# ZhangYY12345/aswStereoMatch

Measured on AMD Instinct MI355X. Metric: disparity Mpix/s, 1920x1080 D=128 classic bilateral ASW (computeAdaptiveWeight), higher is better.
Workload: dtype f64; 1 GPU; 1920x1080 D=128 win=15 bilateral, 8 frames/GPU/step resident in HBM, cost volume kept; candidates=129, parallelism=frames sharded, no collective, ranks=1, backend=none

## Files before the change

### aswstereomatch_amd/csrc/k_bilateral_xq.hip

```cpp
#include <stdlib.h>

#include <algorithm>
#include <cmath>

#include "asw_device.h"
#include "asw_internal.h"

namespace {

constexpr int HH = 7;
constexpr int KS = 2 * HH + 1;
constexpr int PXW = 64;
constexpr int LWC = PXW + 2 * HH;
constexpr int NSTEP = KS + 3;
constexpr int RING = 5;
constexpr int URI = 3;
constexpr int CROW = 6;
static_assert(KS % URI == 0 && CROW % URI == 0, "whole bodies");
constexpr int NCELLCOL = NSTEP + 3;
constexpr int LW8 = 80;
constexpr int LWP = 80;

template <int NW>
struct XqCfg {
    static constexpr int NWAVE = NW;
    static constexpr int NTHR = 64 * NW;
    static constexpr int NJ = 4 * NW;
    static constexpr int NPOS = PXW + 4 * NJ;
    static constexpr int RWC = NPOS + 2 * HH;
    static constexpr int NFIN = 4 * NJ;
    static constexpr int RW8 = (RWC + 3) / 4 * 4;
    static constexpr int NROWS = (KS + NW - 1) / NW;
    static constexpr int RWP = (RWC + 3) / 4 * 4;
    static constexpr int LROW = RING * PXW + LWP;
    static constexpr int RROW = 2 * NPOS + RWP;
    static constexpr int LGRAY = RING * PXW;
    static constexpr int RGRAY = 2 * NPOS;
    static constexpr int OFF_LB = 0;
    static constexpr int OFF_RB = OFF_LB + KS * LROW * 4;
    static constexpr int OFF_L8 = OFF_RB + KS * RROW * 4;
    static constexpr int OFF_R8 = OFF_L8 + KS * LW8;
    static constexpr int OFF_CELL = OFF_R8 + KS * RW8;
    static constexpr int OFF_E64 = 0;
    static constexpr int OFF_PART = (NFIN + 1) * PXW * 8;
    static constexpr int LDS_TOTAL = std::max((OFF_CELL + NCELLCOL * KS * 2 + 15) / 16 * 16, OFF_PART + NW * PXW * 12);
    static_assert(LDS_TOTAL <= (NW == 8 ? 80 : 53) * 1024, "two (NW = 8) / three (NW = 4) workgroups per CU");
    static_assert(OFF_RB % 16 == 0 && (LROW * 4) % 16 == 0 && (RROW * 4) % 16 == 0 && (NPOS * 4) % 16 == 0 && (LGRAY * 4) % 16 == 0, "b128 alignment");
    static_assert(NPOS % 64 == 0, "positions are staged in whole wavefront passes");
};
#define XQ_CONSTS(NW)                                                                                                           \
    typedef XqCfg<NW> Cfg;                                                                                                       \
    constexpr int NWAVE = Cfg::NWAVE, NTHR = Cfg::NTHR, NJ = Cfg::NJ, NPOS = Cfg::NPOS, RWC = Cfg::RWC, NFIN = Cfg::NFIN, RW8 = Cfg::RW8,      \
                  NROWS = Cfg::NROWS, LROW = Cfg::LROW, RROW = Cfg::RROW, LGRAY = Cfg::LGRAY, RGRAY = Cfg::RGRAY,               \
                  OFF_LB = Cfg::OFF_LB, OFF_RB = Cfg::OFF_RB, OFF_L8 = Cfg::OFF_L8, OFF_R8 = Cfg::OFF_R8, OFF_CELL = Cfg::OFF_CELL,  \
                  LDS_TOTAL = Cfg::LDS_TOTAL, OFF_E64 = Cfg::OFF_E64, OFF_PART = Cfg::OFF_PART;                                  \
    (void)NWAVE; (void)NTHR; (void)NJ; (void)NPOS; (void)RWC; (void)NFIN; (void)RW8; (void)NROWS; (void)LROW; (void)RROW; (void)LGRAY;  \
    (void)RGRAY; (void)OFF_LB; (void)OFF_RB; (void)OFF_L8; (void)OFF_R8; (void)OFF_CELL; (void)LDS_TOTAL; (void)OFF_E64; (void)OFF_PART;

struct XqParams {
    int H, W, minD;
    int tile0;
};

__device__ __forceinline__ double cost_sample(uint32_t gl, uint32_t gr, uint32_t hi0)
{
    const uint32_t c = __builtin_amdgcn_sad_u16(gl, gr, 0u);
    return __builtin_bit_cast(double, (uint64_t)c | ((uint64_t)hi0 << 32));
}

template <int NW>
__device__ __forceinline__ void cell_at(const unsigned char* smem, int idx, int& dxw, int& dyw, int& cls256)
{
    XQ_CONSTS(NW)
    const uint32_t u = reinterpret_cast<const uint16_t*>(smem + OFF_CELL)[idx];
    dxw = (int)(u & 15u) - 8;
    dyw = (int)((u >> 4) & 15u) - 8;
    cls256 = (int)(u >> 8) << 8;
}

template <int NW> struct Staged { float v[XqCfg<NW>::NROWS][1 + XqCfg<NW>::NPOS / 64]; };

template <int NW>
__device__ __forceinline__ void stage_issue(int Kn, const float* __restrict__ lut, const unsigned char* smem, int wave, int lane,
                                            uint32_t ppack, Staged<NW>& st)
{
    XQ_CONSTS(NW)
    const uint8_t* sL8 = smem + OFF_L8;
    const uint8_t* sR8 = smem + OFF_R8;
#pragma unroll
    for (int rr = 0; rr < NROWS; rr++) {
        const int ky = wave + NWAVE * rr;
        if (ky >= KS) break;
        int dxw, dyw, cls;
        if (Kn < KS) {
            cell_at<NW>(smem, (Kn + 3) * KS + ky, dxw, dyw, cls);
            const int nb = sL8[(HH + dyw) * LW8 + (lane + HH + dxw)];
            st.v[rr][0] = lut_at(lut, __builtin_amdgcn_sad_u16(nb, sL8[HH * LW8 + lane + HH], cls));
        }
#pragma unroll
        for (int r3 = 0; r3 < NPOS / 64; r3++) {
            const int b = lane & 3;
            cell_at<NW>(smem, (Kn - b + 3) * KS + ky, dxw, dyw, cls);
            const int pc = (int)((ppack >> (8 * r3)) & 255u) + HH;
            const int ctr = sR8[HH * RW8 + pc];
            const int nb = sR8[(HH + dyw) * RW8 + pc + dxw];
            st.v[rr][1 + r3] = lut_at(lut, __builtin_amdgcn_sad_u16(nb, ctr, cls));
        }
    }
}

template <int NW>
__device__ __forceinline__ void stage_commit(int Kn, unsigned char* smem, int wave, int lane, const Staged<NW>& st)
{
    XQ_CONSTS(NW)
    float* sWL = reinterpret_cast<float*>(smem + OFF_LB) + (Kn % RING) * PXW;
    float* sWR = reinterpret_cast<float*>(smem + OFF_RB) + (Kn & 1) * NPOS;
#pragma unroll
    for (int rr = 0; rr < NROWS; rr++) {
        const int ky = wave + NWAVE * rr;
        if (ky >= KS) break;
        if (Kn < KS) sWL[ky * LROW + lane] = st.v[rr][0];
#pragma unroll
        for (int r3 = 0; r3 < NPOS / 64; r3++) sWR[ky * RROW + lane + 64 * r3] = st.v[rr][1 + r3];
    }
}

template <int NW>
__device__ __forceinline__ void stage_weights(int Kn, const float* __restrict__ lut, unsigned char* smem, int wave, int lane,
                                              uint32_t ppack)
{
    Staged<NW> st;
    stage_issue<NW>(Kn, lut, smem, wave, lane, ppack, st);
    stage_commit<NW>(Kn, smem, wave, lane, st);
}

__device__ __forceinline__ int fresh_lane()
{
    int l;
    asm volatile("v_mbcnt_lo_u32_b32 %0, -1, 0\n\tv_mbcnt_hi_u32_b32 %0, -1, %0" : "=&v"(l));
    return l;
}
template <int NPOS>
__device__ __forceinline__ uint32_t pack_positions(int lane, int pclamp_lo, int pclamp_hi)
{
    uint32_t ppack = 0;
#pragma unroll
    for (int r3 = 0; r3 < NPOS / 64; r3++) ppack |= (uint32_t)min(max(lane + 64 * r3, pclamp_lo), pclamp_hi) << (8 * r3);
    asm volatile("" : "+v"(ppack));
    return ppack;
}
template <int NW> constexpr int UWAVE = NW - 1;
template <bool ON> struct USums {};
template <> struct USums<true> { double num = 0.0, den = 0.0; };

template <int NW, int K, bool EDGE, bool WRAPW, bool COMMIT, bool RIGHT, bool LASTW, bool FRESH>
__device__ __forceinline__ void run_step(unsigned char* smem, int g, int qrel, int qrel2, int xabs, int dbase, int dbase2,
                                         int W, int x0, int posmin, double (&num)[4][4], double (&den)[4][4], USums<LASTW>& us,
                                         int wave, int lane, const Staged<NW>& st)
{
    static_assert(!LASTW || (!EDGE && !WRAPW), "the last-candidate units live in a plain wavefront of an interior tile");
    XQ_CONSTS(NW)
    constexpr int BLO = K > KS - 1 ? K - (KS - 1) : 0;
    constexpr int BHI = K < 3 ? K : 3;
    constexpr int DLO = 0 - BHI, DHI = 3 - BLO;
    const uint32_t* sLd = reinterpret_cast<const uint32_t*>(smem + OFF_LB) + LGRAY;
    const uint32_t* sRd = reinterpret_cast<const uint32_t*>(smem + OFF_RB) + RGRAY;

    int iL[7], iR[7];
    if constexpr (EDGE) {
#pragma unroll
        for (int dl = DLO; dl <= DHI; dl++) {
            const int lc = min(max(xabs + dl + K - HH, 0), W - 1);
            const int rc = RIGHT ? lc + ((dl > 0 ? dbase2 : dbase) - dl) : lc - ((dl < 0 ? dbase2 : dbase) + dl);
            iL[dl + 3] = min(max(lc - (x0 - HH), 0), LWC - 1);
            iR[dl + 3] = min(max(rc - (posmin - HH), 0), RWC - 1);
        }
    }
    typedef __attribute__((address_space(3))) const unsigned char lds_u8;
    lds_u8* bL = (lds_u8*)smem + OFF_LB + 16 * g;
    lds_u8* bR = (lds_u8*)smem + OFF_RB + 4 * qrel;
    lds_u8* bR2 = (lds_u8*)smem + OFF_RB + 4 * qrel2;
    lds_u8* uL = nullptr; lds_u8* uW = nullptr; lds_u8* uG = nullptr;
    if constexpr (FRESH) {
        static_assert(!EDGE, "interior tiles");
        const int l2 = fresh_lane();
        g = (l2 & 7) | ((l2 >> 2) & 8);
        const int jl = 4 * wave + ((l2 >> 3) & 3);
        qrel = RIGHT ? 4 * g + 4 * jl : 4 * g + 4 * (NJ - jl);
        qrel2 = jl == 0 ? (RIGHT ? 4 * g + 4 * NJ : 4 * g) : qrel;
        bL = (lds_u8*)smem + OFF_LB + 16 * g;
        bR = (lds_u8*)smem + OFF_RB + 4 * qrel;
        bR2 = (lds_u8*)smem + OFF_RB + 4 * qrel2;
    }
    if constexpr (LASTW) {
        static_assert(FRESH, "g is this step's own");
        const int a = (fresh_lane() >> 3) & 3;
        const int slot = a == 0 ? (K + RING) % RING : a == 1 ? (K - 1 + RING) % RING : a == 2 ? (K - 2 + RING) % RING : (K - 3 + RING) % RING;
        uL = (lds_u8*)smem + OFF_LB + 16 * g + 4 * a + 4 * PXW * slot;
        uW = (lds_u8*)smem + OFF_RB + 16 * g + (RIGHT ? 16 * NJ : 0) + 4 * a + 4 * (K & 1) * NPOS;
        uG = (lds_u8*)smem + OFF_RB + 16 * g + (RIGHT ? 16 * NJ : 0);
        asm("" : "+v"(uL), "+v"(uW), "+v"(uG));
    }
    uint32_t hi0[7];
#pragma unroll
    for (int i = 0; i < 7; i++) asm volatile("v_mov_b32 %0, 0" : "=v"(hi0[i]));
    constexpr int UR = EDGE ? 1 : URI;
    auto rows = [&](int ky0, int nbody) {
#pragma unroll 1
        for (int it = 0; it < nbody; it++) {
#pragma unroll
            for (int u = 0; u < UR; u++) {
                lds_u8* rL = bL + u * 4 * LROW;
                lds_u8* rR = bR + u * 4 * RROW;
                lds_u8* rR2 = bR2 + u * 4 * RROW;
                double c[7];
                uint32_t glU = 0;
                (void)glU;
                if constexpr (!EDGE) {
                    const uint32_t gr = *(const __attribute__((address_space(3))) uint32_t*)(rR + 4 * (RGRAY + K));
                    uint32_t gr2 = gr;
                    if constexpr (WRAPW && (RIGHT ? DHI > 0 : DLO < 0)) gr2 = *(const __attribute__((address_space(3))) uint32_t*)(rR2 + 4 * (RGRAY + K));
                    constexpr int E0 = (K + DLO) & ~3, NQ = (K + DHI - E0 + 4) / 4;
                    static_assert(E0 >= 0 && E0 + 4 * NQ + 4 * 15 <= LWP, "the quads stay inside a tile row");
                    typedef uint32_t u32x4 __attribute__((ext_vector_type(4)));
                    const __attribute__((address_space(3))) u32x4* pl4 = (const __attribute__((address_space(3))) u32x4*)(rL + 4 * (LGRAY + E0));
                    uint32_t glv[4 * NQ];
#pragma unroll
                    for (int i = 0; i < NQ; i++) {
                        u32x4 t = pl4[i];
                        asm("" : "+v"(t));
                        glv[4 * i] = t.x; glv[4 * i + 1] = t.y; glv[4 * i + 2] = t.z; glv[4 * i + 3] = t.w;
                    }
#pragma unroll
                    for (int dl = DLO; dl <= DHI; dl++) c[dl + 3] = cost_sample(glv[K + dl - E0], (RIGHT ? dl > 0 : dl < 0) ? gr2 : gr, hi0[dl + 3]);
                    static_assert(DLO <= 0 && DHI >= 0, "diagonal 0 is in use in every step");
                    glU = glv[K - E0];
                } else {
                    const int ky = ky0 + it * UR + u;
#pragma unroll
                    for (int dl = DLO; dl <= DHI; dl++) c[dl + 3] = cost_sample(sLd[ky * LROW + iL[dl + 3]], sRd[ky * RROW + iR[dl + 3]], hi0[dl + 3]);
                }
                typedef float f32x4 __attribute__((ext_vector_type(4)));
                typedef __attribute__((address_space(3))) const f32x4 lds_f32x4;
                const f32x4 wr4 = *(lds_f32x4*)(rR + 4 * (K & 1) * NPOS);
                typedef float f32x2 __attribute__((ext_vector_type(2)));
                f32x2 wrp[2] = {{wr4.x, wr4.y}, {wr4.z, wr4.w}};
                asm("" : "+v"(wrp[1]));
                f32x2 wr2p[2] = {wrp[0], wrp[1]};
                if constexpr ((WRAPW || EDGE) && (RIGHT ? BLO <= 2 : BHI >= 1)) {
                    const f32x4 w2 = *(lds_f32x4*)(rR2 + 4 * (K & 1) * NPOS);
                    wr2p[0] = f32x2{w2.x, w2.y};
                    wr2p[1] = f32x2{w2.z, w2.w};
                    asm("" : "+v"(wr2p[1]));
                }
#pragma unroll
                for (int b = BLO; b <= BHI; b++) {
                    const f32x4 wl4 = *(lds_f32x4*)(rL + 4 * ((K - b) % RING) * PXW);
                    float ab[4];
#pragma unroll
                    for (int a = 0; a < 4; a += 2) {
                        const f32x2 wl2 = {wl4[a], wl4[a + 1]};
                        const bool w0 = RIGHT ? b < a : a < b, w1 = RIGHT ? b < a + 1 : a + 1 < b;
                        const f32x2 s0 = (w0 ? wr2p : wrp)[b >> 1], s1 = (w1 ? wr2p : wrp)[b >> 1];
                        f32x2 wrb;
                        if (w0 == w1) wrb = (b & 1) ? __builtin_shufflevector(s0, s0, 1, 1) : __builtin_shufflevector(s0, s0, 0, 0);
                        else wrb = f32x2{s0[b & 1], s1[b & 1]};
                        const f32x2 pr = wl2 * wrb;
                        ab[a] = pr.x; ab[a + 1] = pr.y;
                    }
#pragma unroll
                    for (int a = 0; a < 4; a++) {
                        const double abd = (double)ab[a];
                        num[a][b] = __builtin_fma(abd, c[a - b + 3], num[a][b]);
                        den[a][b] = den[a][b] + abd;
                    }
                }
                if constexpr (LASTW) {
                    constexpr int E0 = (K + DLO) & ~3;
                    (void)E0;
                    typedef __attribute__((address_space(3))) const uint32_t lds_u32;
                    typedef __attribute__((address_space(3))) const float lds_f32;
                    const float wlU = *(lds_f32*)(uL + u * 4 * LROW);
                    const float wrU = *(lds_f32*)(uW + u * 4 * RROW);
                    const uint32_t grU = *(lds_u32*)(uG + u * 4 * RROW + 4 * (RGRAY + K));
                    const double abU = (double)(wlU * wrU);
                    us.num = __builtin_fma(abU, cost_sample(glU, grU, hi0[3]), us.num);
                    us.den = us.den + abU;
                    asm volatile("" :: "v"(us.num), "v"(us.den));
                }
#pragma unroll
                for (int b = BLO; b <= BHI; b++)
                    asm volatile("" :: "v"(num[0][b]), "v"(num[1][b]), "v"(num[2][b]), "v"(num[3][b]),
                                       "v"(den[0][b]), "v"(den[1][b]), "v"(den[2][b]), "v"(den[3][b]) : "memory");
                __builtin_amdgcn_sched_barrier(0);
            }
            bL += UR * 4 * LROW;
            bR += UR * 4 * RROW;
            asm("" : "+v"(bL), "+v"(bR));
            if constexpr (WRAPW || EDGE) {
                bR2 += UR * 4 * RROW;
                asm("" : "+v"(bR2));
            }
            if constexpr (LASTW) {
                uL += UR * 4 * LROW;
                uW += UR * 4 * RROW;
                uG += UR * 4 * RROW;
                asm("" : "+v"(uL), "+v"(uW), "+v"(uG));
            }
        }
    };
    if constexpr (COMMIT) {
        rows(0, CROW / UR);
        stage_commit<NW>(K + 1, smem, wave, FRESH ? fresh_lane() : lane, st);
        rows(CROW, (KS - CROW) / UR);
    } else {
        rows(0, KS / UR);
    }
}

template <int NW, bool EDGE, bool WRAPW, int ABL, bool RIGHT, bool LASTW = false, bool FRESH = false>
__device__ __forceinline__ void run_all_steps(unsigned char* smem, const float* __restrict__ lut, int wave, int lane,
                                              uint32_t ppack, int g, int qrel, int qrel2, int xabs, int dbase, int dbase2,
                                              int W, int x0, int posmin, double (&num)[4][4], double (&den)[4][4], USums<LASTW>& us, int pclamp_lo = 0,
                                              int pclamp_hi = 0)
{
    Staged<NW> st;
#define ASW_XQ_STEP(KK)                                                                                        \
    if (!(ABL & 1) && (KK) + 1 < NSTEP) {                                                                        \
        if constexpr (FRESH) { lane = fresh_lane(); ppack = pack_positions<XqCfg<NW>::NPOS>(lane, pclamp_lo, pclamp_hi); }  \
        if constexpr (EDGE) stage_weights<NW>((KK) + 1, lut, smem, wave, lane, ppack);   \
        else stage_issue<NW>((KK) + 1, lut, smem, wave, lane, ppack, st);                      \
    }                                                                                                           \
    run_step<NW, (KK), EDGE, WRAPW, (!EDGE && !(ABL & 1) && (KK) + 1 < NSTEP), RIGHT, LASTW, FRESH>(smem, g, qrel, qrel2, xabs, dbase, dbase2, W, x0, \
                                                                           posmin, num, den, us, wave, lane, st); \
    if (!(ABL & 2) || (KK) == NSTEP - 1) __syncthreads();
    ASW_XQ_STEP(0) ASW_XQ_STEP(1) ASW_XQ_STEP(2) ASW_XQ_STEP(3) ASW_XQ_STEP(4) ASW_XQ_STEP(5)
    ASW_XQ_STEP(6) ASW_XQ_STEP(7) ASW_XQ_STEP(8) ASW_XQ_STEP(9) ASW_XQ_STEP(10) ASW_XQ_STEP(11)
    ASW_XQ_STEP(12) ASW_XQ_STEP(13) ASW_XQ_STEP(14) ASW_XQ_STEP(15) ASW_XQ_STEP(16) ASW_XQ_STEP(17)
#undef ASW_XQ_STEP
}

template <int NW, bool EDGE, int ABL, bool RIGHT, bool LASTC = false>
__global__ __launch_bounds__(64 * NW) __attribute__((amdgpu_waves_per_eu(NW == 8 ? 4 : 3, NW == 8 ? 4 : 3))) void k_asw_bilateral_xq(
    XqParams p, const uint8_t* __restrict__ gL, const uint8_t* __restrict__ gR, const int4* __restrict__ cells,
    const float* __restrict__ lut, float* __restrict__ vol, double* __restrict__ bestE, float* __restrict__ bestD,
    float* __restrict__ disp)
{
    XQ_CONSTS(NW)
    static_assert(!(EDGE && LASTC), "the border tiles cannot host the last-candidate units");
    __shared__ __align__(16) unsigned char smem[LDS_TOTAL];
    const int tid = threadIdx.x, lane = tid & 63, wave = __builtin_amdgcn_readfirstlane(tid >> 6);
    const int H = p.H, W = p.W;
    const int x0 = (p.tile0 + blockIdx.x) * PXW, y = blockIdx.y;
    const int posmin = RIGHT ? x0 + p.minD : x0 - p.minD - 4 * NJ;

    {
        uint8_t* sL8 = smem + OFF_L8;
        uint8_t* sR8 = smem + OFF_R8;
        uint32_t* sLd = reinterpret_cast<uint32_t*>(smem + OFF_LB) + Cfg::LGRAY;
        uint32_t* sRd = reinterpret_cast<uint32_t*>(smem + OFF_RB) + Cfg::RGRAY;
        for (int i = tid; i < KS * LWC; i += NTHR) {
            const int r = i / LWC, c = i - r * LWC;
            const int yy = min(max(y - HH + r, 0), H - 1), xx = min(max(x0 - HH + c, 0), W - 1);
            const int v = gL[(size_t)yy * W + xx];
            sL8[r * LW8 + c] = (uint8_t)v;
            sLd[r * Cfg::LROW + c] = (uint32_t)v;
        }
        for (int i = tid; i < KS * RWC; i += NTHR) {
            const int r = i / RWC, c = i - r * RWC;
            const int yy = min(max(y - HH + r, 0), H - 1), xx = min(max(posmin - HH + c, 0), W - 1);
            const int v = gR[(size_t)yy * W + xx];
            sR8[r * RW8 + c] = (uint8_t)v;
            sRd[r * Cfg::RROW + c] = (uint32_t)v;
        }
        if constexpr (LASTC) {
            float* sWL = reinterpret_cast<float*>(smem + OFF_LB);
            for (int i = tid; i < KS * 3 * PXW; i += NTHR) {
                const int r = i / (3 * PXW), c = i - r * (3 * PXW);
                sWL[r * Cfg::LROW + 2 * PXW + c] = 0.0f;
            }
        }
        uint16_t* sCell = reinterpret_cast<uint16_t*>(smem + OFF_CELL);
        for (int i = tid; i < NCELLCOL * KS; i += NTHR) {
            const int4 ci = cells[i];
            sCell[i] = (uint16_t)((uint32_t)(ci.x + 8) | ((uint32_t)(ci.y + 8) << 4) | ((uint32_t)(ci.z >> 8) << 8));
        }
    }
    __syncthreads();

    const int g = (lane & 7) | ((lane >> 2) & 8);
    const int jl = 4 * wave + ((lane >> 3) & 3);
    const int qrel = RIGHT ? 4 * g + 4 * jl : 4 * g + 4 * (NJ - jl);
    const int qrel2 = jl == 0 ? (RIGHT ? 4 * g + 4 * NJ : 4 * g) : qrel;
    const int xabs = x0 + 4 * g;
    const int dbase = p.minD + 4 * jl;
    const int dbase2 = jl == 0 ? p.minD + 4 * NJ : dbase;
    const int pclamp_lo = min(max(0 - posmin, 0), NPOS - 1), pclamp_hi = min(max(W - 1 - posmin, 0), NPOS - 1);
    static_assert(NPOS <= 256, "a clamped position fits a byte");
    const uint32_t ppack = pack_positions<NPOS>(lane, pclamp_lo, pclamp_hi);

    double num[4][4], den[4][4];
#pragma unroll
    for (int a = 0; a < 4; a++)
#pragma unroll
        for (int b = 0; b < 4; b++) { num[a][b] = 0.0; den[a][b] = 0.0; }

    USums<LASTC> us;
    USums<false> none;
    stage_weights<NW>(0, lut, smem, wave, lane, ppack);
    __syncthreads();
    if (EDGE || wave == 0)
        run_all_steps<NW, EDGE, true, ABL, RIGHT, false, LASTC>(smem, lut, wave, lane, ppack, g, qrel, qrel2, xabs, dbase, dbase2, W,
                                                                 x0, posmin, num, den, none, pclamp_lo, pclamp_hi);
    else if (LASTC && wave == UWAVE<NW>)
        run_all_steps<NW, EDGE, false, ABL, RIGHT, LASTC, LASTC>(smem, lut, UWAVE<NW>, lane, ppack, g, qrel, qrel2, xabs, dbase, dbase2, W,
                                                                  x0, posmin, num, den, us, pclamp_lo, pclamp_hi);
    else
        run_all_steps<NW, EDGE, false, ABL, RIGHT, false, LASTC>(smem, lut, wave, lane, ppack, g, qrel, qrel2, xabs, dbase, dbase2, W,
                                                                  x0, posmin, num, den, none, pclamp_lo, pclamp_hi);

    int le = lane;
    asm volatile("" : "+v"(le));
    const int ge = (le & 7) | ((le >> 2) & 8), jle = 4 * wave + ((le >> 3) & 3);
    const int cb = 4 * jle, cb2 = jle == 0 ? 4 * NJ : cb;
    double* sE = reinterpret_cast<double*>(smem + OFF_E64);
#pragma unroll
    for (int a = 0; a < 4; a++)
#pragma unroll
        for (int b = 0; b < 4; b++) {
            const int c = RIGHT ? (b < a ? cb2 : cb) + b - a : (a < b ? cb2 : cb) + a - b;
            sE[c * PXW + 4 * ge + a] = __builtin_ldexp(num[a][b], 954) / __builtin_ldexp(den[a][b], -120);
        }
    if constexpr (LASTC)
        if (wave == UWAVE<NW>) sE[NFIN * PXW + 4 * ge + ((le >> 3) & 3)] = __builtin_ldexp(us.num, 954) / __builtin_ldexp(us.den, -120);
    __syncthreads();
    const int px = lane, part = wave;
    const int x = x0 + px;
    double be = 1.7976931348623157e308;
    float bd = 0.0f;
    if (x < W) {
        for (int c = 16 * part; c < 16 * part + 16; c++) {
            const double E = sE[c * PXW + px];
            if (vol) vol[((size_t)c * H + y) * W + x] = (float)E;
            if (E < be) { be = E; bd = (float)(p.minD + c); }
        }
    }
    double* sPE = reinterpret_cast<double*>(smem + OFF_PART);
    float* sPD = reinterpret_cast<float*>(smem + OFF_PART + NWAVE * PXW * 8);
    sPE[part * PXW + px] = be;
    sPD[part * PXW + px] = bd;
    __syncthreads();
    if (wave == 0 && x < W) {
        double e = 1.7976931348623157e308;
        float d = 0.0f;
#pragma unroll
        for (int q = 0; q < NWAVE; q++) {
            const double eq = sPE[q * PXW + px];
            if (eq < e) { e = eq; d = sPD[q * PXW + px]; }
        }
        if constexpr (LASTC) {
            const double eq = sE[NFIN * PXW + px];
            if (vol) vol[((size_t)NFIN * H + y) * W + x] = (float)eq;
            if (eq < e) { e = eq; d = (float)(p.minD + NFIN); }
        }
        if (LASTC || disp) {
            disp[(size_t)y * W + x] = d;
        } else {
            bestE[(size_t)y * W + x] = e;
            bestD[(size_t)y * W + x] = d;
        }
    }
}

}

int bilateral_xq_candidates(int nwave) { return 16 * nwave; }

bool bilateral_xq_lut_ok(const float* lut, size_t n)
{
    double mn = 0, mx = 0;
    for (size_t i = 0; i < n; i++) {
        const double v = lut[i];
        if (!(v >= 0)) return false;
        if (v > 0 && (mn == 0 || v < mn)) mn = v;
        if (v > mx) mx = v;
    }
    return mn * mn >= std::ldexp(1.0, -68) && mx * mx < std::ldexp(1.0, 128 - 2 * XQ_LUT_SCALE_LOG2 - 1);
}

namespace {
template <int NW>
int launch_xq_t(hipStream_t s, hipStream_t s_border, const uint8_t* gL, const uint8_t* gR, int H, int W, int minD, const int4* cells,
                const float* lut, float* vol, double* bestE, float* bestD, float* disp, bool right, bool last)
{
    const int ntiles = (W + PXW - 1) / PXW;
    const dim3 blk(64 * NW);
    if (right) {
        if ((ntiles - 1) * PXW + minD > W - 1) return ASW_ERR_BAD_ARGUMENT;
        XqParams pe{H, W, minD, 0};
        hipLaunchKernelGGL((k_asw_bilateral_xq<NW, true, 0, true>), dim3(1, H), blk, 0, s_border, pe, gL, gR, cells, lut, vol,
                           bestE, bestD, last ? nullptr : disp);
        if (ntiles > 1) {
            XqParams pi{H, W, minD, 1};
            if (last)
                hipLaunchKernelGGL((k_asw_bilateral_xq<NW, false, 0, true, true>), dim3(ntiles - 1, H), blk, 0, s, pi, gL, gR, cells,
                                   lut, vol, bestE, bestD, disp);
            else
                hipLaunchKernelGGL((k_asw_bilateral_xq<NW, false, 0, true>), dim3(ntiles - 1, H), blk, 0, s, pi, gL, gR, cells, lut,
                                   vol, bestE, bestD, disp);
        }
        ASW_HIP_TRY(hipGetLastError());
        return ASW_OK;
    }
    const int n_int = W >= PXW + HH ? std::min(ntiles, (W - PXW - HH) / PXW + 1) : 0;
#ifdef ASW_XQ_ABLATION
    int abl = 0;
    if (const char* e = getenv("ASW_XQ_ABLATE")) abl = atoi(e) & 3;
    auto ki = abl == 0 ? k_asw_bilateral_xq<NW, false, 0, false> : abl == 1 ? k_asw_bilateral_xq<NW, false, 1, false>
            : abl == 2 ? k_asw_bilateral_xq<NW, false, 2, false> : k_asw_bilateral_xq<NW, false, 3, false>;
#else
    auto ki = k_asw_bilateral_xq<NW, false, 0, false>;
#endif
    auto ke = k_asw_bilateral_xq<NW, true, 0, false>;
    if (n_int > 0) {
        XqParams p{H, W, minD, 0};
        if (last)
            hipLaunchKernelGGL((k_asw_bilateral_xq<NW, false, 0, false, true>), dim3(n_int, H), blk, 0, s, p, gL, gR, cells, lut, vol,
                               bestE, bestD, disp);
        else
            hipLaunchKernelGGL(ki, dim3(n_int, H), blk, 0, s, p, gL, gR, cells, lut, vol, bestE, bestD, disp);
    }
    if (ntiles > n_int) {
        XqParams p{H, W, minD, n_int};
        hipLaunchKernelGGL(ke, dim3(ntiles - n_int, H), blk, 0, s_border, p, gL, gR, cells, lut, vol, bestE, bestD,
                           last ? nullptr : disp);
    }
    ASW_HIP_TRY(hipGetLastError());
    return ASW_OK;
}
}

int launch_bilateral_xq(hipStream_t s, hipStream_t s_border, int nwave, const uint8_t* gL, const uint8_t* gR, int H, int W, int minD,
                        const int4* cells, const float* lut, float* vol, double* bestE, float* bestD, float* disp, bool right, bool last)
{
    if (last && !disp) return ASW_ERR_BAD_ARGUMENT;
    if (nwave == 8) return launch_xq_t<8>(s, s_border, gL, gR, H, W, minD, cells, lut, vol, bestE, bestD, disp, right, last);
    if (nwave == 4) return launch_xq_t<4>(s, s_border, gL, gR, H, W, minD, cells, lut, vol, bestE, bestD, disp, right, last);
    return ASW_ERR_BAD_ARGUMENT;
}

void bilateral_xq_interior_columns(int W, bool right, int* lo, int* hi)
{
    const int ntiles = (W + PXW - 1) / PXW;
    if (right) {
        *lo = ntiles > 1 ? PXW : W; *hi = W;
    } else {
        const int n_int = W >= PXW + HH ? std::min(ntiles, (W - PXW - HH) / PXW + 1) : 0;
        *lo = 0; *hi = std::min(W, n_int * PXW);
    }
}
```

Baseline: 250.7 Mpix/s.

## Precompute cell offsets and per-lane tables in LDS to cut staging ALU and registers

Cell entries now hold precomputed left/right LDS offsets (32-bit) in place of packed dx/dy nibbles, so weight staging needs no address arithmetic. Per-lane clamped positions, skews and fresh-lane base offsets move into small LDS tables, replacing the ppack register and the repeated recomputation after fresh_lane. The tile prologue loads rows per wave into registers before writing them to LDS, which lets global loads overlap. This adds LDS footprint and extra LDS reads in exchange for fewer VALU ops and less register pressure in the hot loop.

```diff
diff --git a/aswstereomatch_amd/csrc/k_bilateral_xq.hip b/aswstereomatch_amd/csrc/k_bilateral_xq.hip
--- a/aswstereomatch_amd/csrc/k_bilateral_xq.hip
+++ b/aswstereomatch_amd/csrc/k_bilateral_xq.hip
@@ -40,22 +40,28 @@
     static constexpr int OFF_RB = OFF_LB + KS * LROW * 4;
     static constexpr int OFF_L8 = OFF_RB + KS * RROW * 4;
     static constexpr int OFF_R8 = OFF_L8 + KS * LW8;
-    static constexpr int OFF_CELL = OFF_R8 + KS * RW8;
+    static constexpr int OFF_LANE = OFF_R8 + KS * RW8;
+    static constexpr int OFF_BASE = OFF_LANE + 4 * 64;
+    static constexpr int OFF_CELL = OFF_BASE + 3 * 64 * 2;
+    static constexpr int OFF_STEP_END = OFF_CELL + NCELLCOL * KS * 4;
     static constexpr int OFF_E64 = 0;
     static constexpr int OFF_PART = (NFIN + 1) * PXW * 8;
-    static constexpr int LDS_TOTAL = std::max((OFF_CELL + NCELLCOL * KS * 2 + 15) / 16 * 16, OFF_PART + NW * PXW * 12);
+    static constexpr int LDS_TOTAL = std::max((OFF_STEP_END + 15) / 16 * 16, OFF_PART + NW * PXW * 12);
     static_assert(LDS_TOTAL <= (NW == 8 ? 80 : 53) * 1024, "two (NW = 8) / three (NW = 4) workgroups per CU");
     static_assert(OFF_RB % 16 == 0 && (LROW * 4) % 16 == 0 && (RROW * 4) % 16 == 0 && (NPOS * 4) % 16 == 0 && (LGRAY * 4) % 16 == 0, "b128 alignment");
-    static_assert(NPOS % 64 == 0, "positions are staged in whole wavefront passes");
+    static_assert(NPOS % 64 == 0 && NPOS / 64 <= 3, "positions are staged in whole wavefront passes; three columns of the lane table");
+    static_assert(OFF_CELL % 4 == 0 && OFF_BASE % 2 == 0 && OFF_CELL < 65536 && OFF_RB + 4 * NPOS < 65536, "table alignment; offset fields; u16 bases");
+    static_assert((2 * HH) * LW8 + 2 * HH < (1 << 11) && (2 * HH) * RW8 + 2 * HH < (1 << 12), "cell entry fields");
 };
 #define XQ_CONSTS(NW)                                                                                                           \
     typedef XqCfg<NW> Cfg;                                                                                                       \
     constexpr int NWAVE = Cfg::NWAVE, NTHR = Cfg::NTHR, NJ = Cfg::NJ, NPOS = Cfg::NPOS, RWC = Cfg::RWC, NFIN = Cfg::NFIN, RW8 = Cfg::RW8,      \
                   NROWS = Cfg::NROWS, LROW = Cfg::LROW, RROW = Cfg::RROW, LGRAY = Cfg::LGRAY, RGRAY = Cfg::RGRAY,               \
                   OFF_LB = Cfg::OFF_LB, OFF_RB = Cfg::OFF_RB, OFF_L8 = Cfg::OFF_L8, OFF_R8 = Cfg::OFF_R8, OFF_CELL = Cfg::OFF_CELL,  \
+                  OFF_LANE = Cfg::OFF_LANE, OFF_BASE = Cfg::OFF_BASE,                                                            \
                   LDS_TOTAL = Cfg::LDS_TOTAL, OFF_E64 = Cfg::OFF_E64, OFF_PART = Cfg::OFF_PART;                                  \
     (void)NWAVE; (void)NTHR; (void)NJ; (void)NPOS; (void)RWC; (void)NFIN; (void)RW8; (void)NROWS; (void)LROW; (void)RROW; (void)LGRAY;  \
-    (void)RGRAY; (void)OFF_LB; (void)OFF_RB; (void)OFF_L8; (void)OFF_R8; (void)OFF_CELL; (void)LDS_TOTAL; (void)OFF_E64; (void)OFF_PART;
+    (void)RGRAY; (void)OFF_LB; (void)OFF_RB; (void)OFF_L8; (void)OFF_R8; (void)OFF_CELL; (void)OFF_LANE; (void)OFF_BASE; (void)LDS_TOTAL; (void)OFF_E64; (void)OFF_PART;
 
 struct XqParams {
     int H, W, minD;
@@ -68,43 +74,47 @@
     return __builtin_bit_cast(double, (uint64_t)c | ((uint64_t)hi0 << 32));
 }
 
-template <int NW>
-__device__ __forceinline__ void cell_at(const unsigned char* smem, int idx, int& dxw, int& dyw, int& cls256)
-{
-    XQ_CONSTS(NW)
-    const uint32_t u = reinterpret_cast<const uint16_t*>(smem + OFF_CELL)[idx];
-    dxw = (int)(u & 15u) - 8;
-    dyw = (int)((u >> 4) & 15u) - 8;
-    cls256 = (int)(u >> 8) << 8;
+__host__ __device__ constexpr uint32_t cell_entry(int dxw, int dyw, int cls256, int RW8)
+{
+    const uint32_t loff = (uint32_t)((HH + dyw) * LW8 + HH + dxw), roff = (uint32_t)((HH + dyw) * RW8 + HH + dxw);
+    return (loff & 255u) | (uint32_t)cls256 | ((loff >> 8) << 16) | (roff << 20);
 }
 
 template <int NW> struct Staged { float v[XqCfg<NW>::NROWS][1 + XqCfg<NW>::NPOS / 64]; };
 
 template <int NW>
 __device__ __forceinline__ void stage_issue(int Kn, const float* __restrict__ lut, const unsigned char* smem, int wave, int lane,
-                                            uint32_t ppack, Staged<NW>& st)
+                                            Staged<NW>& st)
 {
     XQ_CONSTS(NW)
     const uint8_t* sL8 = smem + OFF_L8;
     const uint8_t* sR8 = smem + OFF_R8;
+    const uint8_t* sLane = smem + OFF_LANE;
+    int pc[NPOS / 64], ctr[NPOS / 64];
+#pragma unroll
+    for (int r3 = 0; r3 < NPOS / 64; r3++) pc[r3] = sLane[64 * r3 + lane];
+    const int skew = sLane[64 * 3 + lane];
+#pragma unroll
+    for (int r3 = 0; r3 < NPOS / 64; r3++) ctr[r3] = sR8[HH * RW8 + HH + pc[r3]];
+    const int ctrL = Kn < KS ? sL8[HH * LW8 + HH + lane] : 0;
+    typedef __attribute__((address_space(3))) const unsigned char lds_u8;
+    lds_u8* pcell = (lds_u8*)smem + OFF_CELL + 4 * ((Kn + 3) * KS + wave) - skew;
+    asm("" : "+v"(pcell));
 #pragma unroll
     for (int rr = 0; rr < NROWS; rr++) {
         const int ky = wave + NWAVE * rr;
         if (ky >= KS) break;
-        int dxw, dyw, cls;
+        const uint32_t u = *(const __attribute__((address_space(3))) uint32_t*)(pcell + 4 * NWAVE * rr);
         if (Kn < KS) {
-            cell_at<NW>(smem, (Kn + 3) * KS + ky, dxw, dyw, cls);
-            const int nb = sL8[(HH + dyw) * LW8 + (lane + HH + dxw)];
-            st.v[rr][0] = lut_at(lut, __builtin_amdgcn_sad_u16(nb, sL8[HH * LW8 + lane + HH], cls));
-        }
+            const uint32_t u0 = (uint32_t)__builtin_amdgcn_readfirstlane((int)u);
+            const int nb = sL8[((u0 & 255u) | ((u0 >> 8) & 0x700u)) + lane];
+            st.v[rr][0] = lut_at(lut, __builtin_amdgcn_sad_u16(nb, ctrL, u0 & 0xff00u));
+        }
+        const int roff = (int)(u >> 20), cls = (int)(u & 0xff00u);
 #pragma unroll
         for (int r3 = 0; r3 < NPOS / 64; r3++) {
-            const int b = lane & 3;
-            cell_at<NW>(smem, (Kn - b + 3) * KS + ky, dxw, dyw, cls);
-            const int pc = (int)((ppack >> (8 * r3)) & 255u) + HH;
-            const int ctr = sR8[HH * RW8 + pc];
-            const int nb = sR8[(HH + dyw) * RW8 + pc + dxw];
-            st.v[rr][1 + r3] = lut_at(lut, __builtin_amdgcn_sad_u16(nb, ctr, cls));
+            const int nb = sR8[roff + pc[r3]];
+            st.v[rr][1 + r3] = lut_at(lut, __builtin_amdgcn_sad_u16(nb, ctr[r3], cls));
         }
     }
 }
@@ -113,24 +123,27 @@
 __device__ __forceinline__ void stage_commit(int Kn, unsigned char* smem, int wave, int lane, const Staged<NW>& st)
 {
     XQ_CONSTS(NW)
-    float* sWL = reinterpret_cast<float*>(smem + OFF_LB) + (Kn % RING) * PXW;
-    float* sWR = reinterpret_cast<float*>(smem + OFF_RB) + (Kn & 1) * NPOS;
+    typedef __attribute__((address_space(3))) float lds_f32;
+    typedef __attribute__((address_space(3))) unsigned char lds_u8w;
+    lds_u8w* cL = (lds_u8w*)smem + 4 * LROW * wave + 4 * lane;
+    lds_u8w* cR = (lds_u8w*)smem + 4 * RROW * wave + 4 * lane + OFF_RB % 256;
+    asm("" : "+v"(cL), "+v"(cR));
 #pragma unroll
     for (int rr = 0; rr < NROWS; rr++) {
         const int ky = wave + NWAVE * rr;
         if (ky >= KS) break;
-        if (Kn < KS) sWL[ky * LROW + lane] = st.v[rr][0];
-#pragma unroll
-        for (int r3 = 0; r3 < NPOS / 64; r3++) sWR[ky * RROW + lane + 64 * r3] = st.v[rr][1 + r3];
+        if (Kn < KS) *(lds_f32*)(cL + OFF_LB + 4 * (Kn % RING) * PXW + 4 * LROW * NWAVE * rr) = st.v[rr][0];
+#pragma unroll
+        for (int r3 = 0; r3 < NPOS / 64; r3++)
+            *(lds_f32*)(cR + (OFF_RB - OFF_RB % 256) + 4 * (Kn & 1) * NPOS + 4 * RROW * NWAVE * rr + 4 * 64 * r3) = st.v[rr][1 + r3];
     }
 }
 
 template <int NW>
-__device__ __forceinline__ void stage_weights(int Kn, const float* __restrict__ lut, unsigned char* smem, int wave, int lane,
-                                              uint32_t ppack)
+__device__ __forceinline__ void stage_weights(int Kn, const float* __restrict__ lut, unsigned char* smem, int wave, int lane)
 {
     Staged<NW> st;
-    stage_issue<NW>(Kn, lut, smem, wave, lane, ppack, st);
+    stage_issue<NW>(Kn, lut, smem, wave, lane, st);
     stage_commit<NW>(Kn, smem, wave, lane, st);
 }
 
@@ -139,15 +152,6 @@
     int l;
     asm volatile("v_mbcnt_lo_u32_b32 %0, -1, 0\n\tv_mbcnt_hi_u32_b32 %0, -1, %0" : "=&v"(l));
     return l;
-}
-template <int NPOS>
-__device__ __forceinline__ uint32_t pack_positions(int lane, int pclamp_lo, int pclamp_hi)
-{
-    uint32_t ppack = 0;
-#pragma unroll
-    for (int r3 = 0; r3 < NPOS / 64; r3++) ppack |= (uint32_t)min(max(lane + 64 * r3, pclamp_lo), pclamp_hi) << (8 * r3);
-    asm volatile("" : "+v"(ppack));
-    return ppack;
 }
 template <int NW> constexpr int UWAVE = NW - 1;
 template <bool ON> struct USums {};
@@ -183,18 +187,16 @@
     lds_u8* uL = nullptr; lds_u8* uW = nullptr; lds_u8* uG = nullptr;
     if constexpr (FRESH) {
         static_assert(!EDGE, "interior tiles");
-        const int l2 = fresh_lane();
-        g = (l2 & 7) | ((l2 >> 2) & 8);
-        const int jl = 4 * wave + ((l2 >> 3) & 3);
-        qrel = RIGHT ? 4 * g + 4 * jl : 4 * g + 4 * (NJ - jl);
-        qrel2 = jl == 0 ? (RIGHT ? 4 * g + 4 * NJ : 4 * g) : qrel;
-        bL = (lds_u8*)smem + OFF_LB + 16 * g;
-        bR = (lds_u8*)smem + OFF_RB + 4 * qrel;
-        bR2 = (lds_u8*)smem + OFF_RB + 4 * qrel2;
+        const uint16_t* sBase = reinterpret_cast<const uint16_t*>(smem + OFF_BASE);
+        const int oL = sBase[lane], oR = sBase[64 + lane] + (RIGHT ? 64 : -64) * wave;
+        bL = (lds_u8*)smem + oL;
+        bR = (lds_u8*)smem + oR;
+        bR2 = WRAPW ? (lds_u8*)smem + sBase[128 + lane] : bR;
+        g = (oL - OFF_LB) >> 4;
     }
     if constexpr (LASTW) {
         static_assert(FRESH, "g is this step's own");
-        const int a = (fresh_lane() >> 3) & 3;
+        const int a = (lane >> 3) & 3;
         const int slot = a == 0 ? (K + RING) % RING : a == 1 ? (K - 1 + RING) % RING : a == 2 ? (K - 2 + RING) % RING : (K - 3 + RING) % RING;
         uL = (lds_u8*)smem + OFF_LB + 16 * g + 4 * a + 4 * PXW * slot;
         uW = (lds_u8*)smem + OFF_RB + 16 * g + (RIGHT ? 16 * NJ : 0) + 4 * a + 4 * (K & 1) * NPOS;
@@ -320,16 +322,15 @@
 
 template <int NW, bool EDGE, bool WRAPW, int ABL, bool RIGHT, bool LASTW = false, bool FRESH = false>
 __device__ __forceinline__ void run_all_steps(unsigned char* smem, const float* __restrict__ lut, int wave, int lane,
-                                              uint32_t ppack, int g, int qrel, int qrel2, int xabs, int dbase, int dbase2,
-                                              int W, int x0, int posmin, double (&num)[4][4], double (&den)[4][4], USums<LASTW>& us, int pclamp_lo = 0,
-                                              int pclamp_hi = 0)
+                                              int g, int qrel, int qrel2, int xabs, int dbase, int dbase2,
+                                              int W, int x0, int posmin, double (&num)[4][4], double (&den)[4][4], USums<LASTW>& us)
 {
     Staged<NW> st;
 #define ASW_XQ_STEP(KK)                                                                                        \
+    if constexpr (FRESH) lane = fresh_lane();                \
     if (!(ABL & 1) && (KK) + 1 < NSTEP) {                                                                        \
-        if constexpr (FRESH) { lane = fresh_lane(); ppack = pack_positions<XqCfg<NW>::NPOS>(lane, pclamp_lo, pclamp_hi); }  \
-        if constexpr (EDGE) stage_weights<NW>((KK) + 1, lut, smem, wave, lane, ppack);   \
-        else stage_issue<NW>((KK) + 1, lut, smem, wave, lane, ppack, st);                      \
+        if constexpr (EDGE) stage_weights<NW>((KK) + 1, lut, smem, wave, lane);   \
+        else stage_issue<NW>((KK) + 1, lut, smem, wave, lane, st);                             \
     }                                                                                                           \
     run_step<NW, (KK), EDGE, WRAPW, (!EDGE && !(ABL & 1) && (KK) + 1 < NSTEP), RIGHT, LASTW, FRESH>(smem, g, qrel, qrel2, xabs, dbase, dbase2, W, x0, \
                                                                            posmin, num, den, us, wave, lane, st); \
@@ -359,31 +360,67 @@
         uint8_t* sR8 = smem + OFF_R8;
         uint32_t* sLd = reinterpret_cast<uint32_t*>(smem + OFF_LB) + Cfg::LGRAY;
         uint32_t* sRd = reinterpret_cast<uint32_t*>(smem + OFF_RB) + Cfg::RGRAY;
-        for (int i = tid; i < KS * LWC; i += NTHR) {
-            const int r = i / LWC, c = i - r * LWC;
-            const int yy = min(max(y - HH + r, 0), H - 1), xx = min(max(x0 - HH + c, 0), W - 1);
-            const int v = gL[(size_t)yy * W + xx];
-            sL8[r * LW8 + c] = (uint8_t)v;
-            sLd[r * Cfg::LROW + c] = (uint32_t)v;
-        }
-        for (int i = tid; i < KS * RWC; i += NTHR) {
-            const int r = i / RWC, c = i - r * RWC;
-            const int yy = min(max(y - HH + r, 0), H - 1), xx = min(max(posmin - HH + c, 0), W - 1);
-            const int v = gR[(size_t)yy * W + xx];
-            sR8[r * RW8 + c] = (uint8_t)v;
-            sRd[r * Cfg::RROW + c] = (uint32_t)v;
-        }
-        if constexpr (LASTC) {
-            float* sWL = reinterpret_cast<float*>(smem + OFF_LB);
-            for (int i = tid; i < KS * 3 * PXW; i += NTHR) {
-                const int r = i / (3 * PXW), c = i - r * (3 * PXW);
-                sWL[r * Cfg::LROW + 2 * PXW + c] = 0.0f;
-            }
-        }
-        uint16_t* sCell = reinterpret_cast<uint16_t*>(smem + OFF_CELL);
-        for (int i = tid; i < NCELLCOL * KS; i += NTHR) {
-            const int4 ci = cells[i];
-            sCell[i] = (uint16_t)((uint32_t)(ci.x + 8) | ((uint32_t)(ci.y + 8) << 4) | ((uint32_t)(ci.z >> 8) << 8));
+        constexpr int NCL = (LWC + 63) / 64, NCR = (RWC + 63) / 64, NCI = (NCELLCOL * KS + NTHR - 1) / NTHR;
+        uint32_t vL[NROWS][NCL], vR[NROWS][NCR];
+        int4 ci[NCI];
+#pragma unroll
+        for (int k = 0; k < NCI; k++) ci[k] = cells[min(tid + NTHR * k, NCELLCOL * KS - 1)];
+#pragma unroll
+        for (int rr = 0; rr < NROWS; rr++) {
+            const int yy = min(max(y - HH + wave + NWAVE * rr, 0), H - 1);
+            const uint8_t* rowL = gL + (size_t)yy * W;
+            const uint8_t* rowR = gR + (size_t)yy * W;
+#pragma unroll
+            for (int k = 0; k < NCL; k++) vL[rr][k] = rowL[min(max(x0 - HH + lane + 64 * k, 0), W - 1)];
+#pragma unroll
+            for (int k = 0; k < NCR; k++) vR[rr][k] = rowR[min(max(posmin - HH + lane + 64 * k, 0), W - 1)];
+        }
+#pragma unroll
+        for (int rr = 0; rr < NROWS; rr++) {
+            const int r = wave + NWAVE * rr;
+            if (r >= KS) break;
+#pragma unroll
+            for (int k = 0; k < NCL; k++) {
+                const int c = lane + 64 * k;
+                if (c < LWC) {
+                    sL8[r * LW8 + c] = (uint8_t)vL[rr][k];
+                    sLd[r * Cfg::LROW + c] = vL[rr][k];
+                }
+            }
+#pragma unroll
+            for (int k = 0; k < NCR; k++) {
+                const int c = lane + 64 * k;
+                if (c < RWC) {
+                    sR8[r * RW8 + c] = (uint8_t)vR[rr][k];
+                    sRd[r * Cfg::RROW + c] = vR[rr][k];
+                }
+            }
+            if constexpr (LASTC) {
+                float* sWL = reinterpret_cast<float*>(smem + OFF_LB);
+#pragma unroll
+                for (int k = 0; k < 3; k++) sWL[r * Cfg::LROW + 2 * PXW + lane + 64 * k] = 0.0f;
+            }
+        }
+        uint32_t* sCell = reinterpret_cast<uint32_t*>(smem + OFF_CELL);
+#pragma unroll
+        for (int k = 0; k < NCI; k++)
+            if (tid + NTHR * k < NCELLCOL * KS) sCell[tid + NTHR * k] = cell_entry(ci[k].x, ci[k].y, ci[k].z, RW8);
+        if (tid < 64) {
+            const int pclamp_lo = min(max(0 - posmin, 0), NPOS - 1), pclamp_hi = min(max(W - 1 - posmin, 0), NPOS - 1);
+            static_assert(NPOS <= 256 && 4 * KS * 3 < 256, "a clamped position and a skew fit a byte");
+            uint8_t* sLane = smem + OFF_LANE;
+#pragma unroll
+            for (int r3 = 0; r3 < NPOS / 64; r3++) sLane[64 * r3 + tid] = (uint8_t)min(max(tid + 64 * r3, pclamp_lo), pclamp_hi);
+            sLane[64 * 3 + tid] = (uint8_t)(4 * KS * (tid & 3));
+            if constexpr (LASTC) {
+                const int g0 = (tid & 7) | ((tid >> 2) & 8), j0 = (tid >> 3) & 3;
+                const int q0 = RIGHT ? 4 * g0 + 4 * j0 : 4 * g0 + 4 * (NJ - j0);
+                const int q2 = j0 == 0 ? (RIGHT ? 4 * g0 + 4 * NJ : 4 * g0) : q0;
+                uint16_t* sBase = reinterpret_cast<uint16_t*>(smem + OFF_BASE);
+                sBase[tid] = (uint16_t)(OFF_LB + 16 * g0);
+                sBase[64 + tid] = (uint16_t)(OFF_RB + 4 * q0);
+                sBase[128 + tid] = (uint16_t)(OFF_RB + 4 * q2);
+            }
         }
     }
     __syncthreads();
@@ -395,9 +432,6 @@
     const int xabs = x0 + 4 * g;
     const int dbase = p.minD + 4 * jl;
     const int dbase2 = jl == 0 ? p.minD + 4 * NJ : dbase;
-    const int pclamp_lo = min(max(0 - posmin, 0), NPOS - 1), pclamp_hi = min(max(W - 1 - posmin, 0), NPOS - 1);
-    static_assert(NPOS <= 256, "a clamped position fits a byte");
-    const uint32_t ppack = pack_positions<NPOS>(lane, pclamp_lo, pclamp_hi);
 
     double num[4][4], den[4][4];
 #pragma unroll
@@ -407,17 +441,17 @@
 
     USums<LASTC> us;
     USums<false> none;
-    stage_weights<NW>(0, lut, smem, wave, lane, ppack);
+    stage_weights<NW>(0, lut, smem, wave, lane);
     __syncthreads();
     if (EDGE || wave == 0)
-        run_all_steps<NW, EDGE, true, ABL, RIGHT, false, LASTC>(smem, lut, wave, lane, ppack, g, qrel, qrel2, xabs, dbase, dbase2, W,
-                                                                 x0, posmin, num, den, none, pclamp_lo, pclamp_hi);
+        run_all_steps<NW, EDGE, true, ABL, RIGHT, false, LASTC>(smem, lut, wave, lane, g, qrel, qrel2, xabs, dbase, dbase2, W,
+                                                                 x0, posmin, num, den, none);
     else if (LASTC && wave == UWAVE<NW>)
-        run_all_steps<NW, EDGE, false, ABL, RIGHT, LASTC, LASTC>(smem, lut, UWAVE<NW>, lane, ppack, g, qrel, qrel2, xabs, dbase, dbase2, W,
-                                                                  x0, posmin, num, den, us, pclamp_lo, pclamp_hi);
+        run_all_steps<NW, EDGE, false, ABL, RIGHT, LASTC, LASTC>(smem, lut, UWAVE<NW>, lane, g, qrel, qrel2, xabs, dbase, dbase2, W,
+                                                                  x0, posmin, num, den, us);
     else
-        run_all_steps<NW, EDGE, false, ABL, RIGHT, false, LASTC>(smem, lut, wave, lane, ppack, g, qrel, qrel2, xabs, dbase, dbase2, W,
-                                                                  x0, posmin, num, den, none, pclamp_lo, pclamp_hi);
+        run_all_steps<NW, EDGE, false, ABL, RIGHT, false, LASTC>(smem, lut, wave, lane, g, qrel, qrel2, xabs, dbase, dbase2, W,
+                                                                  x0, posmin, num, den, none);
 
     int le = lane;
     asm volatile("" : "+v"(le));
```

Result: faster. 254.7 Mpix/s (median of 6 runs) (+1.6%).
